# foldl/chatllm.cpp

Measured on AMD Instinct MI355X. Metric: decode tokens/s, higher is better.
Workload: dtype int8xint4 dot / f32 accumulate (Q8_K x Q4_K); 1 GPU; llama3-8b shapes, Q4_K weights, single-token decode, batch 1, 16-token prompt, F16 KV cache; parallelism=single GPU, n_ctx_end=1630

## Files before the change

chatllm.cpp_amd/csrc/common.h:

```cpp
#pragma once

#include <hip/hip_runtime.h>
#include <stdint.h>
#include <stddef.h>

#include "../../include/chatllm_hip.h"
#include "glibc_math.h"
#include "options.h"

#define CLLM_WAVE 64

void cllm_set_error(const char * fmt, ...);
int  cllm_hip_check(hipError_t e, const char * what, const char * file, int line);
#define HIP_TRY(expr) do { int _rc = cllm_hip_check((expr), #expr, __FILE__, __LINE__); if (_rc) return _rc; } while (0)
#define LAUNCH_CHECK() HIP_TRY(hipGetLastError())
#define FAIL(code, ...) do { cllm_set_error(__VA_ARGS__); return (code); } while (0)

#define QK    32
#define QK_K  256
struct __attribute__((packed)) block_q4_0 { uint16_t d; uint8_t qs[16]; };
struct __attribute__((packed)) block_q8_0 { uint16_t d; int8_t  qs[32]; };
struct __attribute__((packed)) block_q4_1 { uint16_t d, m; uint8_t qs[16]; };
struct __attribute__((packed)) block_q8_1 { uint16_t d, s; int8_t  qs[32]; };
struct __attribute__((packed)) block_q4_K { uint16_t d, dmin; uint8_t scales[12]; uint8_t qs[128]; };
// ... 178 lines not shown
__device__ __forceinline__ int   group8_sum_i(int v) { v += dpp_i<DPP_QUAD_XOR1>(v); v += dpp_i<DPP_QUAD_XOR2>(v); return v + dpp_i<DPP_HALF_MIRROR>(v); }
__device__ __forceinline__ int dot4(uint32_t a, uint32_t b, int c) { return __builtin_amdgcn_sdot4((int) a, (int) b, c, false); }
__device__ __forceinline__ void dot4z_x8(const uint32_t (&a)[8], const uint32_t (&b)[8], int (&r)[8]) {
    asm("v_dot4_i32_i8 %0, %8, %16, 0\n\tv_dot4_i32_i8 %1, %9, %17, 0\n\tv_dot4_i32_i8 %2, %10, %18, 0\n\tv_dot4_i32_i8 %3, %11, %19, 0\n\t"
        "v_dot4_i32_i8 %4, %12, %20, 0\n\tv_dot4_i32_i8 %5, %13, %21, 0\n\tv_dot4_i32_i8 %6, %14, %22, 0\n\tv_dot4_i32_i8 %7, %15, %23, 0\n\ts_nop 2"
        : "=&v"(r[0]), "=&v"(r[1]), "=&v"(r[2]), "=&v"(r[3]), "=&v"(r[4]), "=&v"(r[5]), "=&v"(r[6]), "=&v"(r[7])
        : "v"(a[0]), "v"(a[1]), "v"(a[2]), "v"(a[3]), "v"(a[4]), "v"(a[5]), "v"(a[6]), "v"(a[7]),
          "v"(b[0]), "v"(b[1]), "v"(b[2]), "v"(b[3]), "v"(b[4]), "v"(b[5]), "v"(b[6]), "v"(b[7]));
}

static __device__ __noinline__ float libm_expf(float x) { return gm_expf(x); }
static __device__ __noinline__ void rope_cos_sin(float theta, float * c, float * s) {
    *c = gm_cosf(theta);
    *s = gm_sinf(theta);
}

__device__ __forceinline__ float rope_rot_a(float x0, float x1, float c, float s) { return __builtin_fmaf(x0, c, -(x1 * s)); }
__device__ __forceinline__ float rope_rot_b(float x0, float x1, float c, float s) { return __builtin_fmaf(x0, s, x1 * c); }

__device__ __forceinline__ float ggml_expf_poly(float x) {
    const float r = 0x1.8p23f;
    const float z = __builtin_fmaf(x, 0x1.715476p+0f, r);
    const float n = z - r;
    const float b = __builtin_fmaf(-n, 0x1.7f7d1cp-20f, __builtin_fmaf(-n, 0x1.62e4p-1f, x));
    const uint32_t e = __float_as_uint(z) << 23;
    const float k = __uint_as_float(e + 0x3f800000u);
    const bool  c = fabsf(n) > 126.0f;
    const float u = b * b;
    const float j = __builtin_fmaf(__builtin_fmaf(__builtin_fmaf(0x1.0e4020p-7f, b, 0x1.573e2ep-5f), u,
                                                  __builtin_fmaf(0x1.555e66p-3f, b, 0x1.fffdb6p-2f)),
// ... 156 lines not shown
int launch_gemv_decode_tp_gather(hipStream_t st, int wtype, const void * W, int64_t K, int64_t nrows, const float * px, const float * pw, float eps, int epi, float * dst,
                                 const float * bias, const void * ctx_dev, int site, float * xout);
int launch_gemv_rows32(hipStream_t st, int wtype, const void * W, int64_t K, int64_t nrows, int pro, const float * px, const float * pw, float eps, int epi, float * dst, const float * bias, const float * resid);
int gemv_team32_check();
int launch_gemv_team32(hipStream_t st, int wtype, const void * W, int64_t K, int64_t nrows, int pro, const float * px, const float * pw, float eps, int epi, float * dst, const float * bias, const float * resid);
int launch_mmvq_fused(hipStream_t st, int wtype, const void * W, int64_t K, int64_t nrows, int pro, const float * px, const float * pw, float eps, int epi, float * dst, const float * bias, const float * resid);
int launch_attn_decode(hipStream_t st, const float * qkv, const int32_t * pos_dev, int nh, int nkv, int hd, const uint16_t * k_cache, const uint16_t * v_cache, int64_t ML, float * att);
int launch_rope_table(hipStream_t st, const int32_t * pos_dev, int hd, float freq_base, float * cs);
int launch_attn_dec_table(hipStream_t st, const float * qkv, const int32_t * pos_dev, const float * rope_cs, int nh, int nkv, int hd, int mode, uint16_t * k_cache, uint16_t * v_cache, int64_t ML, float * att);
int launch_attn_long(hipStream_t st, const float * qkv, const int32_t * pos_dev, const float * rope_cs, int nh, int nkv, int hd, int mode, uint16_t * k_cache, uint16_t * v_cache, int64_t ML, float * S, float * att);
int launch_gemv_decode_id(hipStream_t st, int wtype, const void * W, size_t w_expert_bytes, int64_t K, int64_t nrows, const float * px, int64_t px_slot_stride,
                          const int32_t * ids, int n_slots, float * dst, int64_t dst_slot_stride, int epi = 0);
int attn_long_threshold();
int launch_rope_kv_attn_decode(hipStream_t st, const float * qkv, const int32_t * pos_dev, int nh, int nkv, int hd, int mode, float freq_base, uint16_t * k_cache, uint16_t * v_cache, int64_t ML, float * att);
int launch_argmax_partial(hipStream_t st, const float * logits, int n, float * part_v, int * part_i);
int launch_argmax_final_next(hipStream_t st, const float * part_v, const int * part_i, int np, int32_t * tok_dev, int32_t * pos_dev, int32_t * out_ring, int32_t * counter,
                             int etype, const void * emb, size_t emb_nb1, int H, float * x_next, int hd, float freq_base, float * cs);
int launch_gemv_rows_argmax(hipStream_t st, const void * W, int64_t K, int64_t nrows, const float * px, const float * pw, float eps, float * dst, float * part_v, int * part_i, int * np);
int launch_argmax_advance(hipStream_t st, const float * logits, int n, int32_t * tok_dev, int32_t * pos_dev, int32_t * out_ring, int32_t * counter, float * part_v, int * part_i);
```

chatllm.cpp_amd/csrc/decode_fused.hip:

```cpp
#include "common.h"
#include "quant_dev.h"
#include "q4k.h"
#include "dequant.h"

#include <math.h>

__device__ __forceinline__ float lane_xor4_ff(float v) { return __int_as_float(lane_xor4_i(__float_as_int(v))); }
__device__ __forceinline__ float vd32_reduce(float a0, float a1) {
    a0 = a0 + dpp_f<DPP_ROW_ROR8>(a0); a1 = a1 + dpp_f<DPP_ROW_ROR8>(a1);
    a0 = a0 + lane_xor4_ff(a0);        a1 = a1 + lane_xor4_ff(a1);
    a0 = a0 + dpp_f<DPP_QUAD_XOR2>(a0); a1 = a1 + dpp_f<DPP_QUAD_XOR2>(a1);
    const float u = a0 + a1;
    return u + dpp_f<DPP_QUAD_XOR1>(u);
}

static float * g_attn_dbg = nullptr;
static unsigned long long * g_attn_ts = nullptr;
extern "C" __attribute__((visibility("default"))) void cllm_debug_set_attn_ts(unsigned long long * dev_buf) { g_attn_ts = dev_buf; }
extern "C" __attribute__((visibility("default"))) void cllm_debug_set_attn_probs(float * dev_buf) { g_attn_dbg = dev_buf; }

template <bool ROPE>
__global__ void __launch_bounds__(1024) k_attn_decode(const float * __restrict__ qkv, const int32_t * __restrict__ pos_dev, int nh, int nkv, int hd,
                                                      float scale, uint16_t * __restrict__ k_cache, uint16_t * __restrict__ v_cache,
                                                      int64_t ML, float * __restrict__ att, float * __restrict__ dbg, int mode, float theta_scale) {
// ... 128 lines not shown
        for (int t = 0; t < 2; t++) {
            const int e = np + 2 * c16 + t;
            if (e < n_kv) tailp[2 * c16 + t] = ((ROPE && e == pos) ? vfresh : h2f(vr[e])) * sc[e];
        }
        wave_lds_fence();
        if (c16 == 0) {
            double s = (double) res;
            for (int t = 0; t < ntail; t++) s += (double) tailp[t];
            att[h * hd + d0] = (float) s;
        }
        wave_lds_fence();
    }
}

__global__ void __launch_bounds__(64) k_rope_table(const int32_t * __restrict__ pos_dev, int half, float theta_scale, float * __restrict__ cs) {
    for (int i = threadIdx.x; i < half; i += 64) {
        float theta = (float) pos_dev[0];
        for (int k = 0; k < i; k++) theta *= theta_scale;
        float c, s_;
        rope_cos_sin(theta, &c, &s_);
        cs[2*i] = c * 1.0f; cs[2*i + 1] = s_ * 1.0f;
    }
}
int launch_rope_table(hipStream_t st, const int32_t * pos_dev, int hd, float freq_base, float * cs) {
    hipLaunchKernelGGL(k_rope_table, dim3(1), dim3(64), 0, st, pos_dev, hd / 2, powf(freq_base, -2.0f / hd), cs);
    LAUNCH_CHECK();
    return CLLM_OK;
}

__device__ __forceinline__ int uniform_load_i32(const int32_t * p) {
    int v;
    asm volatile("s_load_dword %0, %1, 0x0\n\ts_waitcnt lgkmcnt(0)" : "=s"(v) : "s"(p) : "memory");
    return v;
}

template <int HD, int MODE, int PARTS>
__global__ void __launch_bounds__(1024) k_attn_dec(const float * __restrict__ qkv, const int32_t * __restrict__ pos_dev, const float * __restrict__ rope_cs,
// ... 10 lines not shown
    float * qs = sm; float * knew = sm + HD; float * vnew = sm + 2 * HD; float * sc = sm + 3 * HD;

    float px0 = 0.0f, px1 = 0.0f, pc = 0.0f, ps = 0.0f;
    const bool is_pair = tid < 2 * half, is_v = !is_pair && tid < 2 * half + HD;
    const int which = tid >= half ? 1 : 0, pi = tid - which * half, ic = MODE == 0 ? 2 * pi : pi;
    if (is_pair) {
        const float * x = which == 0 ? qkv + h * HD : qkv + QD + g * HD;
        px0 = x[ic]; px1 = x[ic + off];
        pc = rope_cs[2 * pi]; ps = rope_cs[2 * pi + 1];
    } else if (is_v) px0 = qkv[QD + KD + g * HD + (tid - 2 * half)];
    const int pos = uniform_load_i32(pos_dev);
    const int n_kv = pos + 1;
    uint64_t et = 0;
    if (tid >= 992) et = gm_exp2f_T_dev[tid - 992];

    constexpr int NCH = HD / 32, VU = HD / 64 / PARTS, VPF = 8;
    const int vrow0 = PARTS > 1 ? (int) blockIdx.z * VU * 64 : 0;
    const int c16 = lane & 15, sub = lane >> 4;
    const int ib0 = wave * 4 + sub;
    uint32_t kr0[U][NCH];
#pragma unroll
    for (int u = 0; u < U; u++) {
        const int i0 = ib0 + u * 64;
#pragma unroll
        for (int i = 0; i < NCH; i++)
            kr0[u][i] = *(const uint32_t *)(k_cache + (int64_t)(i0 < pos ? i0 : 0) * KD + g * HD + 32 * i + 2 * c16);
    }
    const int np = n_kv & ~31, nch = np >> 5;
    uint32_t vc0[VU][VPF];
#pragma unroll
    for (int u = 0; u < VU; u++) {
        const uint16_t * vr = v_cache + ((int64_t) g * HD + vrow0 + ib0 + u * 64) * ML;
#pragma unroll
        for (int i = 0; i < VPF; i++) vc0[u][i] = *(const uint32_t *)(vr + 32 * (i < nch ? i : 0) + 2 * c16);
    }

    TS(0);
    if (is_pair) {
        const float y0 = rope_rot_a(px0, px1, pc, ps), y1 = rope_rot_b(px0, px1, pc, ps);
        float * o = which == 0 ? qs : knew;
        o[ic] = h2f(f2h(y0)); o[ic + off] = h2f(f2h(y1));
    } else if (is_v) vnew[tid - 2 * half] = h2f(f2h(px0));
    if (tid >= 992) etab_s[tid - 992] = et;
    lds_barrier();
    if (blockIdx.x == 0 && (PARTS == 1 || blockIdx.z == 0) && tid < HD) {
        k_cache[(int64_t) pos * KD + g * HD + tid] = f2h(knew[tid]);
        v_cache[((int64_t) g * HD + tid) * ML + pos] = f2h(vnew[tid]);
    }

// ... 23 lines not shown
                if (c16 == 0 && i0 < pos) sc[i0] = v * scale;
            }
            if (ib + U * 64 < pos) {
#pragma unroll
                for (int u = 0; u < U; u++) {
                    const int i0 = ib + (U + u) * 64;
#pragma unroll
                    for (int i = 0; i < NCH; i++) kr0[u][i] = *(const uint32_t *)(k_cache + (int64_t)(i0 < pos ? i0 : 0) * KD + g * HD + 32 * i + 2 * c16);
                }
            }
        }
    }
    lds_barrier();
    TS(2);

    uint32_t vc1[VU][VPF]; uint16_t vtl[VU][2];
#pragma unroll
    for (int u = 0; u < VU; u++) {
        const uint16_t * vr = v_cache + ((int64_t) g * HD + vrow0 + ib0 + u * 64) * ML;
#pragma unroll
        for (int i = 0; i < VPF; i++) vc1[u][i] = *(const uint32_t *)(vr + 32 * (VPF + i < nch ? VPF + i : 0) + 2 * c16);
#pragma unroll
        for (int t = 0; t < 2; t++) { const int e = np + 2 * c16 + t; vtl[u][t] = vr[e < n_kv ? e : 0]; }
    }
    float mx = -INFINITY;
    for (int i = tid; i < n_kv; i += 1024) mx = fmaxf(mx, sc[i]);
    mx = wave_max(mx);
    if (lane == 0) red_f[wave] = mx;
    lds_barrier();
    mx = red_f[0];
#pragma unroll
    for (int w = 1; w < 16; w++) mx = fmaxf(mx, red_f[w]);
    const int nv = n_kv & ~7;
    for (int i = tid; i < n_kv; i += 1024) {
        const float xv = sc[i] - mx;
        float ev;
        if (i < nv) ev = ggml_expf_poly(xv);
        else { const uint64_t ki = gm_expf_ki(xv); ev = gm_expf_fin(xv, ki, etab_s[ki & 31]); }
// ... 9 lines not shown
        }
        if (lane == 0) for (int i = nv; i < n_kv; i++) sum += (double) sc[i];
        sum = wave_sum_d(sum);
        double rinv = 1.0 / sum;
        if (__builtin_expect(!soft_total_order_safe(rinv, n_kv >> 3), 0)) rinv = 1.0 / soft_sum_serial(sc, nv, n_kv);
        if (lane == 0) red_f[0] = (float) rinv;
    }
    lds_barrier();
    const float inv = red_f[0];
    for (int i = tid; i < n_kv; i += 1024) sc[i] = h2f(f2h(sc[i] * inv));
    lds_barrier();
    TS(3);

    float * tailp = sc + ML + (wave * 4 + sub) * 32;
    const int ntail = n_kv - np;
#pragma unroll
    for (int u = 0; u < VU; u++) {
        const int d0 = vrow0 + ib0 + u * 64;
        const uint16_t * vr = v_cache + ((int64_t) g * HD + d0) * ML;
        const float vfresh = vnew[d0];
        float a0 = 0.0f, a1 = 0.0f;
        auto chunk = [&](uint32_t w, int ci) {
            const int e = 32 * ci + 2 * c16;
            typedef float f32x2_t __attribute__((ext_vector_type(2)));
            const f32x2_t pr = *(const f32x2_t *)(sc + e);
            const float v0 = e == pos ? vfresh : h2f((uint16_t)(w & 0xffff)), v1 = e + 1 == pos ? vfresh : h2f((uint16_t)(w >> 16));
            a0 = __builtin_fmaf(v0, pr.x, a0); a1 = __builtin_fmaf(v1, pr.y, a1);
        };
#pragma unroll
        for (int i = 0; i < VPF; i++) if (i < nch) chunk(vc0[u][i], i);
        if (nch > VPF) {
#pragma unroll
            for (int i = 0; i < VPF; i++) if (VPF + i < nch) chunk(vc1[u][i], VPF + i);
#pragma clang loop unroll(disable)
            for (int c8 = 2 * VPF; c8 < nch; c8 += VPF) {
                uint32_t w[VPF];
#pragma unroll
                for (int i = 0; i < VPF; i++) w[i] = *(const uint32_t *)(vr + 32 * (c8 + i < nch ? c8 + i : 0) + 2 * c16);
#pragma unroll
                for (int i = 0; i < VPF; i++) if (c8 + i < nch) chunk(w[i], c8 + i);
            }
        }
        const float res = vd32_reduce(a0, a1);
#pragma unroll
        for (int t = 0; t < 2; t++) {
            const int e = np + 2 * c16 + t;
            if (e < n_kv) tailp[2 * c16 + t] = (e == pos ? vfresh : h2f(vtl[u][t])) * sc[e];
        }
        wave_lds_fence();
        if (c16 == 0) {
            double s = (double) res;
            for (int t = 0; t < ntail; t++) s += (double) tailp[t];
            att[h * HD + d0] = (float) s;
        }
        wave_lds_fence();
    }
    TS(4);
#undef TS
}

int launch_attn_dec_table(hipStream_t st, const float * qkv, const int32_t * pos_dev, const float * rope_cs, int nh, int nkv, int hd, int mode,
                          uint16_t * k_cache, uint16_t * v_cache, int64_t ML, float * att) {
    if ((hd != 64 && hd != 128) || nh % nkv || ML % 8 || ML > (1 << 30) || g_attn_dbg) return CLLM_E_UNSUPPORTED;
    const size_t lds = (size_t)(3 * hd + ML) * 4 + 64 * 32 * 4;
    if (lds > 150 * 1024) return CLLM_E_UNSUPPORTED;
    const float scale = 1.0f / sqrtf((float) hd);
    const dim3 grid(nh / nkv, nkv, hd == 128 ? 2 : 1);
#define GO(HD_, MODE_) do { \
        static uint64_t attr = 0; \
        if (lds > 48 * 1024 && dev_flag_unset(attr)) { HIP_TRY(hipFuncSetAttribute((const void *) k_attn_dec<HD_, MODE_, (HD_ == 128 ? 2 : 1)>, hipFuncAttributeMaxDynamicSharedMemorySize, 150 * 1024)); dev_flag_set(attr); } \
        hipLaunchKernelGGL((k_attn_dec<HD_, MODE_, (HD_ == 128 ? 2 : 1)>), grid, dim3(1024), lds, st, qkv, pos_dev, rope_cs, nh, nkv, scale, k_cache, v_cache, (int) ML, att, g_attn_ts); } while (0)
    if (hd == 128) { if (mode == 0) GO(128, 0); else GO(128, 2); }
    else           { if (mode == 0) GO(64, 0);  else GO(64, 2); }
#undef GO
    LAUNCH_CHECK();
    return CLLM_OK;
}

static int attn_launch(hipStream_t st, bool rope, const float * qkv, const int32_t * pos_dev, int nh, int nkv, int hd, uint16_t * k_cache, uint16_t * v_cache,
                       int64_t ML, float * att, int mode, float freq_base) {
    if (hd % 8 || (ML % 8) || nh % nkv) FAIL(CLLM_E_UNSUPPORTED, "attn_decode: head_dim and max_len must be multiples of 8");
    const size_t lds = (size_t)(3 * hd + (ML > hd ? ML : hd)) * 4 + 64 * 32 * 4;
    if (lds > 150 * 1024) FAIL(CLLM_E_UNSUPPORTED, "attn_decode: max_len %lld does not fit LDS", (long long) ML);
    static uint64_t attr0 = 0, attr1 = 0;
    if (lds > 48 * 1024) {
        if (!rope && dev_flag_unset(attr0)) { HIP_TRY(hipFuncSetAttribute((const void *) k_attn_decode<false>, hipFuncAttributeMaxDynamicSharedMemorySize, 150 * 1024)); dev_flag_set(attr0); }
// ... 75 lines not shown
    float best = -INFINITY; int idx = 0x7fffffff;
    for (int i = threadIdx.x; i < np; i += 256) argmax_combine(best, idx, pv[i], pi[i]);
#pragma unroll
    for (int o = 32; o > 0; o >>= 1) argmax_combine(best, idx, __shfl_xor(best, o, 64), __shfl_xor(idx, o, 64));
    if ((threadIdx.x & 63) == 0) { bv[threadIdx.x >> 6] = best; bi[threadIdx.x >> 6] = idx; }
    __syncthreads();
    if (threadIdx.x == 0) {
        for (int w = 1; w < 4; w++) argmax_combine(best, idx, bv[w], bi[w]);
        if (idx == 0x7fffffff) idx = 0;
        tok_dev[0] = idx;
        pos_dev[0] = pos_dev[0] + 1;
        out_ring[counter[0]] = idx;
        counter[0] = counter[0] + 1;
    }
}
__global__ void __launch_bounds__(1024) k_argmax_final_next(const float * __restrict__ pv, const int * __restrict__ pi, int np, int32_t * __restrict__ tok_dev,
                                                            int32_t * __restrict__ pos_dev, int32_t * __restrict__ out_ring, int32_t * __restrict__ counter,
                                                            int etype, const char * __restrict__ emb, size_t emb_nb1, int H, float * __restrict__ x_next,
                                                            int half, float theta_scale, float * __restrict__ cs) {
    __shared__ float bv[16]; __shared__ int bi[16]; __shared__ int tok_s;
    const int tid = threadIdx.x;
    const int pos_next = pos_dev[0] + 1;
    float best = -INFINITY; int idx = 0x7fffffff;
    for (int i = tid; i < np; i += 1024) argmax_combine(best, idx, pv[i], pi[i]);
#pragma unroll
    for (int o = 32; o > 0; o >>= 1) argmax_combine(best, idx, __shfl_xor(best, o, 64), __shfl_xor(idx, o, 64));
    if ((tid & 63) == 0) { bv[tid >> 6] = best; bi[tid >> 6] = idx; }
    __syncthreads();
    if (tid == 0) {
        for (int w = 1; w < 16; w++) argmax_combine(best, idx, bv[w], bi[w]);
        if (idx == 0x7fffffff) idx = 0;
        tok_s = idx;
        tok_dev[0] = idx;
        pos_dev[0] = pos_next;
        out_ring[counter[0]] = idx;
        counter[0] = counter[0] + 1;
    }
    if (cs && tid >= 960)
        for (int i = tid - 960; i < half; i += 64) {
            float theta = (float) pos_next;
            for (int k = 0; k < i; k++) theta *= theta_scale;
            float c, s_;
            rope_cos_sin(theta, &c, &s_);
            cs[2*i] = c * 1.0f; cs[2*i + 1] = s_ * 1.0f;
        }
    __syncthreads();
    const char * row = emb + (size_t) tok_s * emb_nb1;
    for (int c = tid; c < H; c += 1024) x_next[c] = dequant_elem(etype, row, c);
}
int launch_argmax_partial(hipStream_t st, const float * logits, int n, float * part_v, int * part_i) {
    hipLaunchKernelGGL(k_argmax_partial, dim3(256), dim3(256), 0, st, logits, n, part_v, part_i);
    LAUNCH_CHECK();
    return CLLM_OK;
}
int launch_argmax_final_next(hipStream_t st, const float * part_v, const int * part_i, int np, int32_t * tok_dev, int32_t * pos_dev, int32_t * out_ring, int32_t * counter,
                             int etype, const void * emb, size_t emb_nb1, int H, float * x_next, int hd, float freq_base, float * cs) {
    hipLaunchKernelGGL(k_argmax_final_next, dim3(1), dim3(1024), 0, st, part_v, part_i, np, tok_dev, pos_dev, out_ring, counter, etype, (const char *) emb, emb_nb1, H, x_next,
                       hd / 2, hd ? powf(freq_base, -2.0f / hd) : 0.0f, hd ? cs : (float *) nullptr);
    LAUNCH_CHECK();
    return CLLM_OK;
}
__global__ void __launch_bounds__(256) k_argmax_publish(const float * __restrict__ pv, const int * __restrict__ pi, int np, int32_t * __restrict__ tok_dev,
                                                        int32_t * __restrict__ tok_host, int32_t * const * __restrict__ inc, int n_inc) {
    __shared__ float bv[4]; __shared__ int bi[4];
    float best = -INFINITY; int idx = 0x7fffffff;
    for (int i = threadIdx.x; i < np; i += 256) argmax_combine(best, idx, pv[i], pi[i]);
#pragma unroll
    for (int o = 32; o > 0; o >>= 1) argmax_combine(best, idx, __shfl_xor(best, o, 64), __shfl_xor(idx, o, 64));
    if ((threadIdx.x & 63) == 0) { bv[threadIdx.x >> 6] = best; bi[threadIdx.x >> 6] = idx; }
    __syncthreads();
    if (threadIdx.x == 0) {
        for (int w = 1; w < 4; w++) argmax_combine(best, idx, bv[w], bi[w]);
        if (idx == 0x7fffffff) idx = 0;
// ... 108 lines not shown
```

chatllm.cpp_amd/csrc/decoder.hip:

```cpp
#include "common.h"

#include <string>
#include <vector>
#include <map>
#include <math.h>
#include <string.h>
#include <stdio.h>

struct dweight { int type = -1; void * data = nullptr; size_t bytes = 0; bool owned = false; };

struct llama_layer {
    dweight attn_norm, ffn_norm, wq, wk, wv, wo, wgate, wup, wdown, bq, bk, bv;
    dweight wqkv, wgu;
    dweight bqkv;
    uint16_t * k_cache = nullptr, * v_cache = nullptr;
};

struct cllm_llama {
    cllm_llama_config cfg;
    hipStream_t st = nullptr;
    int nh = 0, nkv = 0, F = 0;
    dweight tok_embd, lm_head, out_norm;
    std::vector<llama_layer> layers;
    bool finalized = false;
// ... 510 lines not shown
        TRY(norm_gemv(L.wgu, 2*F, (const float *) L.ffn_norm.data, silu_epi ? 1 : 0, silu_epi ? m->g : m->gu, nullptr));
        if (!tp) TRY(launch_mmvq_fused(st, L.wdown.type, L.wdown.data, F, H, dpro, dsrc, nullptr, 0.0f, 0, xc, nullptr, xc));
        else if (fused_ar) {
            const int rc = launch_gemv_decode_tp_scatter(st, L.wdown.type, L.wdown.data, F, H, dpro, dsrc, fctx, 2 * il + 1);
            if (rc == CLLM_E_UNSUPPORTED) FAIL(CLLM_E_UNSUPPORTED, "decode: the fused all-reduce cannot take down_proj (type %d, K %lld); unbind it (cllm_llama_set_tp_fused(m, NULL))", L.wdown.type, (long long) F);
            if (rc) return rc;
            pend_site = 2 * il + 1;
        } else {
            TRY(launch_mmvq_fused(st, L.wdown.type, L.wdown.data, F, H, dpro, dsrc, nullptr, 0.0f, 0, m->o, nullptr, nullptr));
            TRY(tp_allreduce(m, st, m->o, H));
            pend = m->o;
        }
    }
    float * part_v = (float *)(m->counter_dev + 16); int * part_i = (int *)(m->counter_dev + 16 + 256);
    if (sample && !head) {
        int np = 256, rc = CLLM_E_UNSUPPORTED;
        if (pend_site < 0 && !pend && m->lm_head.type == CLLM_TYPE_Q4_K)
            rc = launch_gemv_rows_argmax(st, m->lm_head.data, H, V, xc, (const float *) m->out_norm.data, c.rms_eps, m->logits, part_v, part_i, &np);
        if (rc == CLLM_E_UNSUPPORTED) {
            TRY(norm_gemv(m->lm_head, V, (const float *) m->out_norm.data, 0, m->logits, nullptr));
            TRY(launch_argmax_partial(st, m->logits, (int) V, part_v, part_i));
            np = 256;
        } else if (rc) return rc;
        TRY(launch_argmax_final_next(st, part_v, part_i, np, m->tokens_dev, m->pos_dev, m->out_ring, m->counter_dev, m->tok_embd.type, m->tok_embd.data,
                                     cllm_row_size(m->tok_embd.type, H), (int) H, m->x, cs_table ? (int) hd : 0, c.rope_theta, rope_cs));
        return CLLM_OK;
    }
    TRY(norm_gemv(m->lm_head, V, (const float *) m->out_norm.data, 0, m->logits, nullptr));
    if (sample) TRY(launch_argmax_advance(st, m->logits, (int) V, m->tokens_dev, m->pos_dev, m->out_ring, m->counter_dev, part_v, part_i));
    return CLLM_OK;
}

static int kernel_wait_check(cllm_llama * m) {
    TRY(gemv_team32_check());
    if (m->tp_oneshot && cllm_tp_oneshot_error(m->tp_oneshot)) FAIL(CLLM_E_HIP, "decode: a flag wait of the one-shot all-reduce timed out (a peer rank is late, dead or out of step): the step's logits are void");
    if (m->tp_fused && cllm_tp_fused_error(m->tp_fused)) FAIL(CLLM_E_HIP, "decode: a granule wait of the fused all-reduce timed out (a peer rank is late, dead or out of step): the step's logits are void");
    return CLLM_OK;
}

static int ensure_decode_graph(cllm_llama * m, bool long_ctx) {
// ... 92 lines not shown
    if (!m->fused_ok) FAIL(CLLM_E_UNSUPPORTED, "decode_fused_logits: this model/config cannot take the fused path");
    const int32_t init[2] = { token, n_past };
    HIP_TRY(hipMemcpyAsync(m->tokens_dev, &init[0], 4, hipMemcpyHostToDevice, m->st));
    HIP_TRY(hipMemcpyAsync(m->pos_dev, &init[1], 4, hipMemcpyHostToDevice, m->st));
    HIP_TRY(hipStreamSynchronize(m->st));
    TRY(ensure_scores(m, (size_t) m->nh * m->cfg.max_len * 3 / 2 + 64));
    TRY(decode_step_fused(m, false, n_past + 1 > attn_long_threshold()));
    HIP_TRY(hipMemcpyAsync(logits_host, m->logits, (size_t) m->cfg.vocab * 4, hipMemcpyDeviceToHost, m->st));
    HIP_TRY(hipStreamSynchronize(m->st));
    return kernel_wait_check(m);
}

extern "C" int cllm_llama_debug_read(cllm_llama * m, const char * what, float * host, int64_t n) {
    if (!m || !what || !host || n <= 0) FAIL(CLLM_E_INVALID, "debug_read: arguments");
    const std::string w(what);
    const float * src = w == "x" ? m->x : w == "qkv" ? m->qkv : w == "att" ? m->att : w == "gu" ? m->gu : w == "logits" ? m->logits : nullptr;
    if (!src) FAIL(CLLM_E_INVALID, "debug_read: unknown buffer '%s'", what);
    HIP_TRY(hipMemcpyAsync(host, src, (size_t) n * 4, hipMemcpyDeviceToHost, m->st));
    HIP_TRY(hipStreamSynchronize(m->st));
    return CLLM_OK;
}
```

chatllm.cpp_amd/csrc/gemv_rows.hip:

```cpp
#include "common.h"
#include "quant_dev.h"
#include "q4k.h"

#define ROWS_SLOT_BYTES 2304
#ifndef ROWS_NS
#define ROWS_NS 3
#endif

__device__ __forceinline__ float silu_poly_r(float x) { return x / (1.0f + ggml_expf_poly(0.0f - x)); }
__device__ __forceinline__ float silu_any_r(float x, bool body) { return body ? silu_poly_r(x) : x / (1.0f + libm_expf(-x)); }

__device__ __forceinline__ void dma16(const char * base , unsigned voff, unsigned lds_dst ) {
    unsigned keep;
#ifdef ROWS_NT
    asm volatile("s_mov_b32 %0, m0\n\ts_mov_b32 m0, %3\n\ts_nop 0\n\tglobal_load_lds_dwordx4 %1, %2 nt\n\ts_mov_b32 m0, %0" : "=&s"(keep) : "v"(voff), "s"(base), "s"(lds_dst) : "memory");
#else
    asm volatile("s_mov_b32 %0, m0\n\ts_mov_b32 m0, %3\n\ts_nop 0\n\tglobal_load_lds_dwordx4 %1, %2\n\ts_mov_b32 m0, %0" : "=&s"(keep) : "v"(voff), "s"(base), "s"(lds_dst) : "memory");
#endif
}
template <int N> __device__ __forceinline__ void wait_vm() { asm volatile("s_waitcnt vmcnt(%0)" :: "n"(N) : "memory"); }

template <int PRO, int EPI, int NPRE, int RPW>
__global__ void __launch_bounds__(1024) k_gemv_rows(const float * __restrict__ px, const float * __restrict__ pw, const char * __restrict__ W, int nblk, int nunits, float eps,
                                                    float * __restrict__ dst, const float * __restrict__ bias, const float * resid) {
    extern __shared__ __attribute__((aligned(16))) char lds[];
    constexpr int GPR = 8 / RPW;
    constexpr int CPR = ROWS_SLOT_BYTES / RPW / 16;
    constexpr int BPS = 2 * GPR;
    constexpr int NS = ROWS_NS;
    const int tid = threadIdx.x, lane = tid & 63;
    const int K = nblk * 256;
    const unsigned nb01 = (unsigned) nblk * 144u;

    const float * gp = (PRO == 1 || PRO == 4) ? pw : PRO == 3 ? px + 4 : px;
    constexpr int vmul = PRO == 3 ? 2 : 1;
    const int e0 = tid * 4;
    f32x4 vv[NPRE], gg[NPRE];
#pragma unroll
    for (int u = 0; u < NPRE; u++) {
// ... 46 lines not shown
            if (PRO == 3) {
                const f32x4 p0 = vv[u], p1 = gg[u];
                v.x = silu_any_r(p0.x, e + 0 < nv) * p0.y; v.y = silu_any_r(p0.z, e + 1 < nv) * p0.w;
                v.z = silu_any_r(p1.x, e + 2 < nv) * p1.y; v.w = silu_any_r(p1.z, e + 3 < nv) * p1.w;
            }
            if (PRO == 4) {
                const f32x4 g = gg[u];
                v.x = silu_any_r(v.x, e + 0 < nv) * g.x; v.y = silu_any_r(v.y, e + 1 < nv) * g.y; v.z = silu_any_r(v.z, e + 2 < nv) * g.z; v.w = silu_any_r(v.w, e + 3 < nv) * g.w;
            }
            if (PRO == 1) { const f32x4 g = gg[u]; v.x = (v.x * scale) * g.x; v.y = (v.y * scale) * g.y; v.z = (v.z * scale) * g.z; v.w = (v.w * scale) * g.w; }
            quant4_store<256, false>(lds, K, e, lane, v);
        }
    }
    __syncthreads();
    if (EPI != 2 && nmine == 0) return;

    const int j = lane & 7;
    const int A = 4 * (j & 1) + (j & 2) + (j >> 2);
    const int kk = ((j & 1) << 1) | ((j >> 1) & 1);
    const int rowg = RPW == 8 ? lane >> 3 : lane >> 4;
    const int gg2 = RPW == 8 ? 0 : (lane >> 3) & 1;
    const bool hi = gg2 != 0;
    const unsigned lrow = ring + (unsigned) rowg * (CPR * 16u) + (unsigned) gg2 * 144u + 16u + 4u * A;
    const unsigned lhdr = ring + (unsigned) rowg * (CPR * 16u) + (unsigned) gg2 * 144u;
    const char * act = lds;
    const float * actd = (const float *)(lds + act_off_d(K));
    const int * acts = (const int *)(lds + act_off_s(K, 256));
    typedef __attribute__((address_space(3))) const uint32_t * lptr;
    typedef __attribute__((address_space(3))) const u32x4 * lptr4;

// ... 79 lines not shown
            const float ov = __shfl_xor(bestv, o, 64); const int oi = __shfl_xor(besti, o, 64);
            if (ov > bestv || (ov == bestv && oi < besti)) { bestv = ov; besti = oi; }
        }
        __syncthreads();
        float * lv = (float *) lds; int * li = (int *)(lds + 64);
        if (lane == 0) { lv[wave] = bestv; li[wave] = besti; }
        __syncthreads();
        if (tid == 0) {
            for (int w = 1; w < 16; w++) { const float ov = lv[w]; const int oi = li[w]; if (ov > bestv || (ov == bestv && oi < besti)) { bestv = ov; besti = oi; } }
            ((float *) bias)[blockIdx.x] = bestv; ((int *) resid)[blockIdx.x] = besti;
        }
    }
}

static int gemv_rows_go(hipStream_t st, const void * W, int64_t K, int64_t nrows, int pro, const float * px, const float * pw, float eps, int epi, float * dst,
                        const float * bias, const float * resid, int * grid_out) {
    static const int mode = opt_int(OPT_CLLM_GEMV_ROWS);
    if (!mode || K % 256 || pro < 1 || pro > 4 || nrows <= 0 || (uint64_t) nrows * (uint64_t)(K / 256 * 144) >= (1ull << 32)) return CLLM_E_UNSUPPORTED;
    if (K > ((pro == 2 || pro == 4) ? 32768 : 16384)) return CLLM_E_UNSUPPORTED;
    if (epi == 1 && (pro != 1 || bias || resid)) return CLLM_E_UNSUPPORTED;
    if (epi == 2 && (pro != 1 || !bias || !resid)) return CLLM_E_UNSUPPORTED;
    const int nblk = (int)(K / 256), cus = device_cu_count();
    if (mode == 1 && nrows / 8 < 32 * (int64_t) cus) return CLLM_E_UNSUPPORTED;
    int rpw = mode == 8 || mode == 4 ? mode : (nrows / 8 >= 8 * (int64_t) cus ? 8 : 4);
    if (rpw == 8 && (nblk % 2 || nrows % 8)) rpw = 4;
    if (rpw == 4 && (nblk % 4 || nrows % 4)) { if (nblk % 2 == 0 && nrows % 8 == 0) rpw = 8; else return CLLM_E_UNSUPPORTED; }
    if (epi == 1 && nrows % (2 * rpw)) return CLLM_E_UNSUPPORTED;
    const int nunits = (int)(nrows / rpw);
    int grid = nunits < cus ? nunits : cus;
    if (epi == 2 && grid > 256) return CLLM_E_UNSUPPORTED;
    const size_t lds = act_row_bytes(K, 256) + 16 * (size_t) ROWS_NS * ROWS_SLOT_BYTES;
    if (lds > 159 * 1024) return CLLM_E_UNSUPPORTED;
    const int npre = K <= 4096 ? 1 : K <= 16384 ? 4 : 8;
#define GOR(PRO_, EPI_, NPRE_, RPW_) do { \
        static uint64_t attr = 0; \
        if (dev_flag_unset(attr)) { HIP_TRY(hipFuncSetAttribute((const void *) k_gemv_rows<PRO_, EPI_, NPRE_, RPW_>, hipFuncAttributeMaxDynamicSharedMemorySize, 159 * 1024)); dev_flag_set(attr); } \
        hipLaunchKernelGGL((k_gemv_rows<PRO_, EPI_, NPRE_, RPW_>), dim3((unsigned) grid), dim3(1024), lds, st, px, pw, (const char *) W, nblk, nunits, eps, dst, bias, resid); } while (0)
#define GOP(RPW_) do { \
        if (pro == 1 && epi == 1) { if (npre == 1) GOR(1, 1, 1, RPW_); else GOR(1, 1, 4, RPW_); } \
        else if (pro == 1 && epi == 2) { if (npre == 1) GOR(1, 2, 1, RPW_); else GOR(1, 2, 4, RPW_); } \
        else if (pro == 1)        { if (npre == 1) GOR(1, 0, 1, RPW_); else GOR(1, 0, 4, RPW_); } \
        else if (pro == 2)        { if (npre == 1) GOR(2, 0, 1, RPW_); else if (npre == 4) GOR(2, 0, 4, RPW_); else GOR(2, 0, 8, RPW_); } \
        else if (pro == 4)        { if (npre == 1) GOR(4, 0, 1, RPW_); else if (npre == 4) GOR(4, 0, 4, RPW_); else GOR(4, 0, 8, RPW_); } \
        else                      { if (npre == 1) GOR(3, 0, 1, RPW_); else GOR(3, 0, 4, RPW_); } } while (0)
    if (rpw == 8) GOP(8); else GOP(4);
#undef GOP
#undef GOR
    LAUNCH_CHECK();
    if (grid_out) *grid_out = grid;
    return CLLM_OK;
}
int launch_gemv_rows(hipStream_t st, const void * W, int64_t K, int64_t nrows, int pro, const float * px, const float * pw, float eps, int epi, float * dst,
                     const float * bias, const float * resid) {
    if (epi != 0 && epi != 1) return CLLM_E_UNSUPPORTED;
    return gemv_rows_go(st, W, K, nrows, pro, px, pw, eps, epi, dst, bias, resid, nullptr);
}
int launch_gemv_rows_argmax(hipStream_t st, const void * W, int64_t K, int64_t nrows, const float * px, const float * pw, float eps, float * dst, float * part_v, int * part_i, int * np) {
    if (!part_v || !part_i || !np || nrows > INT32_MAX) return CLLM_E_UNSUPPORTED;
    return gemv_rows_go(st, W, K, nrows, 1, px, pw, eps, 2, dst, (const float *) part_v, (const float *) part_i, np);
}
```

Before: 669.2 tokens/s.

## Move next-token rope table into lm_head kernel and split attention into more parts

Builds the next position's rope cos/sin table inside the lm_head gemv-argmax kernel (in the last block's spare wave) or in an extra block of the argmax-partial kernel. This takes it off the serial single-block argmax_final kernel. That kernel is also slimmed: it drops its LDS reduction and barriers, loads partials directly per lane, and specialises on Q4_K embedding dequant. Separately, attention decode for hd=128 splits V rows across 8 parts instead of 2 to spread work over more blocks. The catch is that some waves now sit idle and K/score work is recomputed per part.

```diff
diff --git a/chatllm.cpp_amd/csrc/common.h b/chatllm.cpp_amd/csrc/common.h
--- a/chatllm.cpp_amd/csrc/common.h
+++ b/chatllm.cpp_amd/csrc/common.h
@@ -216,6 +216,16 @@
     *c = gm_cosf(theta);
     *s = gm_sinf(theta);
 }
+__device__ __forceinline__ void rope_table_wave(int pos, int half, float theta_scale, float * __restrict__ cs, int lane) {
+    for (int i = lane; i < half; i += 64) {
+        float theta = (float) pos;
+        for (int k = 0; k < i; k++) theta *= theta_scale;
+        float c, s_;
+        rope_cos_sin(theta, &c, &s_);
+        cs[2*i] = c * 1.0f; cs[2*i + 1] = s_ * 1.0f;
+    }
+}
+struct rope_next { const int32_t * pos_dev; float * cs; int half; float theta_scale; };
 
 __device__ __forceinline__ float rope_rot_a(float x0, float x1, float c, float s) { return __builtin_fmaf(x0, c, -(x1 * s)); }
 __device__ __forceinline__ float rope_rot_b(float x0, float x1, float c, float s) { return __builtin_fmaf(x0, s, x1 * c); }
@@ -402,7 +412,10 @@
 int attn_long_threshold();
 int launch_rope_kv_attn_decode(hipStream_t st, const float * qkv, const int32_t * pos_dev, int nh, int nkv, int hd, int mode, float freq_base, uint16_t * k_cache, uint16_t * v_cache, int64_t ML, float * att);
 int launch_argmax_partial(hipStream_t st, const float * logits, int n, float * part_v, int * part_i);
+rope_next rope_next_args(const int32_t * pos_dev, int hd, float freq_base, float * cs);
+int launch_argmax_partial_next(hipStream_t st, const float * logits, int n, float * part_v, int * part_i, rope_next nx);
 int launch_argmax_final_next(hipStream_t st, const float * part_v, const int * part_i, int np, int32_t * tok_dev, int32_t * pos_dev, int32_t * out_ring, int32_t * counter,
-                             int etype, const void * emb, size_t emb_nb1, int H, float * x_next, int hd, float freq_base, float * cs);
-int launch_gemv_rows_argmax(hipStream_t st, const void * W, int64_t K, int64_t nrows, const float * px, const float * pw, float eps, float * dst, float * part_v, int * part_i, int * np);
+                             int etype, const void * emb, size_t emb_nb1, int H, float * x_next);
+int launch_gemv_rows_argmax(hipStream_t st, const void * W, int64_t K, int64_t nrows, const float * px, const float * pw, float eps, float * dst, float * part_v, int * part_i, int * np,
+                            rope_next nx);
 int launch_argmax_advance(hipStream_t st, const float * logits, int n, int32_t * tok_dev, int32_t * pos_dev, int32_t * out_ring, int32_t * counter, float * part_v, int * part_i);
diff --git a/chatllm.cpp_amd/csrc/decode_fused.hip b/chatllm.cpp_amd/csrc/decode_fused.hip
--- a/chatllm.cpp_amd/csrc/decode_fused.hip
+++ b/chatllm.cpp_amd/csrc/decode_fused.hip
@@ -166,13 +166,7 @@
 }
 
 __global__ void __launch_bounds__(64) k_rope_table(const int32_t * __restrict__ pos_dev, int half, float theta_scale, float * __restrict__ cs) {
-    for (int i = threadIdx.x; i < half; i += 64) {
-        float theta = (float) pos_dev[0];
-        for (int k = 0; k < i; k++) theta *= theta_scale;
-        float c, s_;
-        rope_cos_sin(theta, &c, &s_);
-        cs[2*i] = c * 1.0f; cs[2*i + 1] = s_ * 1.0f;
-    }
+    rope_table_wave(pos_dev[0], half, theta_scale, cs, threadIdx.x);
 }
 int launch_rope_table(hipStream_t st, const int32_t * pos_dev, int hd, float freq_base, float * cs) {
     hipLaunchKernelGGL(k_rope_table, dim3(1), dim3(64), 0, st, pos_dev, hd / 2, powf(freq_base, -2.0f / hd), cs);
@@ -213,8 +207,10 @@
     uint64_t et = 0;
     if (tid >= 992) et = gm_exp2f_T_dev[tid - 992];
 
-    constexpr int NCH = HD / 32, VU = HD / 64 / PARTS, VPF = 8;
-    const int vrow0 = PARTS > 1 ? (int) blockIdx.z * VU * 64 : 0;
+    constexpr int NCH = HD / 32, RP = HD / PARTS, VU = RP >= 64 ? RP / 64 : 1, VPF = RP >= 64 ? 8 : 16;
+    static_assert(RP % 4 == 0 && RP * PARTS == HD && (RP >= 64 ? RP % 64 == 0 : true), "rows per part: whole waves of four lane groups");
+    const int vrow0 = PARTS > 1 ? (int) blockIdx.z * RP : 0;
+    const bool vrow = RP >= 64 || __builtin_amdgcn_readfirstlane(wave) < RP / 4;
     const int c16 = lane & 15, sub = lane >> 4;
     const int ib0 = wave * 4 + sub;
     uint32_t kr0[U][NCH];
@@ -227,11 +223,13 @@
     }
     const int np = n_kv & ~31, nch = np >> 5;
     uint32_t vc0[VU][VPF];
-#pragma unroll
-    for (int u = 0; u < VU; u++) {
-        const uint16_t * vr = v_cache + ((int64_t) g * HD + vrow0 + ib0 + u * 64) * ML;
-#pragma unroll
-        for (int i = 0; i < VPF; i++) vc0[u][i] = *(const uint32_t *)(vr + 32 * (i < nch ? i : 0) + 2 * c16);
+    if (vrow) {
+#pragma unroll
+        for (int u = 0; u < VU; u++) {
+            const uint16_t * vr = v_cache + ((int64_t) g * HD + vrow0 + ib0 + u * 64) * ML;
+#pragma unroll
+            for (int i = 0; i < VPF; i++) vc0[u][i] = *(const uint32_t *)(vr + 32 * (i < nch ? i : 0) + 2 * c16);
+        }
     }
 
     TS(0);
@@ -285,14 +283,19 @@
     lds_barrier();
     TS(2);
 
-    uint32_t vc1[VU][VPF]; uint16_t vtl[VU][2];
-#pragma unroll
-    for (int u = 0; u < VU; u++) {
-        const uint16_t * vr = v_cache + ((int64_t) g * HD + vrow0 + ib0 + u * 64) * ML;
-#pragma unroll
-        for (int i = 0; i < VPF; i++) vc1[u][i] = *(const uint32_t *)(vr + 32 * (VPF + i < nch ? VPF + i : 0) + 2 * c16);
-#pragma unroll
-        for (int t = 0; t < 2; t++) { const int e = np + 2 * c16 + t; vtl[u][t] = vr[e < n_kv ? e : 0]; }
+    constexpr int VPF1 = VPF < 16 ? VPF : 1;
+    uint32_t vc1[VU][VPF1]; uint16_t vtl[VU][2];
+    if (vrow) {
+#pragma unroll
+        for (int u = 0; u < VU; u++) {
+            const uint16_t * vr = v_cache + ((int64_t) g * HD + vrow0 + ib0 + u * 64) * ML;
+            if constexpr (VPF < 16) {
+#pragma unroll
+                for (int i = 0; i < VPF; i++) vc1[u][i] = *(const uint32_t *)(vr + 32 * (VPF + i < nch ? VPF + i : 0) + 2 * c16);
+            }
+#pragma unroll
+            for (int t = 0; t < 2; t++) { const int e = np + 2 * c16 + t; vtl[u][t] = vr[e < n_kv ? e : 0]; }
+        }
     }
     float mx = -INFINITY;
     for (int i = tid; i < n_kv; i += 1024) mx = fmaxf(mx, sc[i]);
@@ -332,6 +335,7 @@
 
     float * tailp = sc + ML + (wave * 4 + sub) * 32;
     const int ntail = n_kv - np;
+    if (vrow) {
 #pragma unroll
     for (int u = 0; u < VU; u++) {
         const int d0 = vrow0 + ib0 + u * 64;
@@ -348,15 +352,17 @@
 #pragma unroll
         for (int i = 0; i < VPF; i++) if (i < nch) chunk(vc0[u][i], i);
         if (nch > VPF) {
-#pragma unroll
-            for (int i = 0; i < VPF; i++) if (VPF + i < nch) chunk(vc1[u][i], VPF + i);
+            if constexpr (VPF < 16) {
+#pragma unroll
+                for (int i = 0; i < VPF; i++) if (VPF + i < nch) chunk(vc1[u][i], VPF + i);
+            }
 #pragma clang loop unroll(disable)
-            for (int c8 = 2 * VPF; c8 < nch; c8 += VPF) {
-                uint32_t w[VPF];
-#pragma unroll
-                for (int i = 0; i < VPF; i++) w[i] = *(const uint32_t *)(vr + 32 * (c8 + i < nch ? c8 + i : 0) + 2 * c16);
-#pragma unroll
-                for (int i = 0; i < VPF; i++) if (c8 + i < nch) chunk(w[i], c8 + i);
+            for (int c8 = 16; c8 < nch; c8 += 8) {
+                uint32_t w[8];
+#pragma unroll
+                for (int i = 0; i < 8; i++) w[i] = *(const uint32_t *)(vr + 32 * (c8 + i < nch ? c8 + i : 0) + 2 * c16);
+#pragma unroll
+                for (int i = 0; i < 8; i++) if (c8 + i < nch) chunk(w[i], c8 + i);
             }
         }
         const float res = vd32_reduce(a0, a1);
@@ -373,21 +379,25 @@
         }
         wave_lds_fence();
     }
+    }
     TS(4);
 #undef TS
 }
 
+#ifndef ATTN_PARTS_128
+#define ATTN_PARTS_128 8
+#endif
 int launch_attn_dec_table(hipStream_t st, const float * qkv, const int32_t * pos_dev, const float * rope_cs, int nh, int nkv, int hd, int mode,
                           uint16_t * k_cache, uint16_t * v_cache, int64_t ML, float * att) {
     if ((hd != 64 && hd != 128) || nh % nkv || ML % 8 || ML > (1 << 30) || g_attn_dbg) return CLLM_E_UNSUPPORTED;
     const size_t lds = (size_t)(3 * hd + ML) * 4 + 64 * 32 * 4;
     if (lds > 150 * 1024) return CLLM_E_UNSUPPORTED;
     const float scale = 1.0f / sqrtf((float) hd);
-    const dim3 grid(nh / nkv, nkv, hd == 128 ? 2 : 1);
+    const dim3 grid(nh / nkv, nkv, hd == 128 ? ATTN_PARTS_128 : 1);
 #define GO(HD_, MODE_) do { \
         static uint64_t attr = 0; \
-        if (lds > 48 * 1024 && dev_flag_unset(attr)) { HIP_TRY(hipFuncSetAttribute((const void *) k_attn_dec<HD_, MODE_, (HD_ == 128 ? 2 : 1)>, hipFuncAttributeMaxDynamicSharedMemorySize, 150 * 1024)); dev_flag_set(attr); } \
-        hipLaunchKernelGGL((k_attn_dec<HD_, MODE_, (HD_ == 128 ? 2 : 1)>), grid, dim3(1024), lds, st, qkv, pos_dev, rope_cs, nh, nkv, scale, k_cache, v_cache, (int) ML, att, g_attn_ts); } while (0)
+        if (lds > 48 * 1024 && dev_flag_unset(attr)) { HIP_TRY(hipFuncSetAttribute((const void *) k_attn_dec<HD_, MODE_, (HD_ == 128 ? ATTN_PARTS_128 : 1)>, hipFuncAttributeMaxDynamicSharedMemorySize, 150 * 1024)); dev_flag_set(attr); } \
+        hipLaunchKernelGGL((k_attn_dec<HD_, MODE_, (HD_ == 128 ? ATTN_PARTS_128 : 1)>), grid, dim3(1024), lds, st, qkv, pos_dev, rope_cs, nh, nkv, scale, k_cache, v_cache, (int) ML, att, g_attn_ts); } while (0)
     if (hd == 128) { if (mode == 0) GO(128, 0); else GO(128, 2); }
     else           { if (mode == 0) GO(64, 0);  else GO(64, 2); }
 #undef GO
@@ -493,39 +503,63 @@
         counter[0] = counter[0] + 1;
     }
 }
+__global__ void __launch_bounds__(256) k_argmax_partial_next(const float * __restrict__ x, int n, float * __restrict__ pv, int * __restrict__ pi, rope_next nx) {
+    __shared__ float bv[4]; __shared__ int bi[4];
+    const int nb = gridDim.x - 1;
+    if ((int) blockIdx.x == nb) {
+        if (threadIdx.x < 64) rope_table_wave(nx.pos_dev[0] + 1, nx.half, nx.theta_scale, nx.cs, threadIdx.x);
+        return;
+    }
+    const int per = (n + nb - 1) / nb;
+    const int lo = blockIdx.x * per, hi = min(n, lo + per);
+    float best = -INFINITY; int idx = 0x7fffffff;
+    for (int i = lo + threadIdx.x; i < hi; i += 256) { const float v = x[i]; if (v > best) { best = v; idx = i; } }
+#pragma unroll
+    for (int o = 32; o > 0; o >>= 1) argmax_combine(best, idx, __shfl_xor(best, o, 64), __shfl_xor(idx, o, 64));
+    if ((threadIdx.x & 63) == 0) { bv[threadIdx.x >> 6] = best; bi[threadIdx.x >> 6] = idx; }
+    __syncthreads();
+    if (threadIdx.x == 0) {
+        for (int w = 1; w < 4; w++) argmax_combine(best, idx, bv[w], bi[w]);
+        pv[blockIdx.x] = best; pi[blockIdx.x] = idx;
+    }
+}
+rope_next rope_next_args(const int32_t * pos_dev, int hd, float freq_base, float * cs) {
+    rope_next nx;
+    nx.pos_dev = pos_dev; nx.cs = hd ? cs : (float *) nullptr; nx.half = hd / 2; nx.theta_scale = hd ? powf(freq_base, -2.0f / hd) : 0.0f;
+    return nx;
+}
+int launch_argmax_partial_next(hipStream_t st, const float * logits, int n, float * part_v, int * part_i, rope_next nx) {
+    if (!nx.cs) return launch_argmax_partial(st, logits, n, part_v, part_i);
+    hipLaunchKernelGGL(k_argmax_partial_next, dim3(257), dim3(256), 0, st, logits, n, part_v, part_i, nx);
+    LAUNCH_CHECK();
+    return CLLM_OK;
+}
+template <int ETYPE>
 __global__ void __launch_bounds__(1024) k_argmax_final_next(const float * __restrict__ pv, const int * __restrict__ pi, int np, int32_t * __restrict__ tok_dev,
                                                             int32_t * __restrict__ pos_dev, int32_t * __restrict__ out_ring, int32_t * __restrict__ counter,
-                                                            int etype, const char * __restrict__ emb, size_t emb_nb1, int H, float * __restrict__ x_next,
-                                                            int half, float theta_scale, float * __restrict__ cs) {
-    __shared__ float bv[16]; __shared__ int bi[16]; __shared__ int tok_s;
-    const int tid = threadIdx.x;
-    const int pos_next = pos_dev[0] + 1;
+                                                            int etype, const char * __restrict__ emb, size_t emb_nb1, int H, float * __restrict__ x_next) {
+    const int tid = threadIdx.x, lane = tid & 63;
+    int pos = 0, cnt = 0;
+    if (tid == 0) { pos = pos_dev[0]; cnt = counter[0]; }
+    float pvv[4]; int pii[4];
+#pragma unroll
+    for (int k = 0; k < 4; k++) { const int i = lane + 64 * k, ic = i < np ? i : 0; pvv[k] = pv[ic]; pii[k] = pi[ic]; }
     float best = -INFINITY; int idx = 0x7fffffff;
-    for (int i = tid; i < np; i += 1024) argmax_combine(best, idx, pv[i], pi[i]);
-#pragma unroll
-    for (int o = 32; o > 0; o >>= 1) argmax_combine(best, idx, __shfl_xor(best, o, 64), __shfl_xor(idx, o, 64));
-    if ((tid & 63) == 0) { bv[tid >> 6] = best; bi[tid >> 6] = idx; }
-    __syncthreads();
+#pragma unroll
+    for (int k = 0; k < 4; k++) if (lane + 64 * k < np) argmax_combine(best, idx, pvv[k], pii[k]);
+#pragma unroll
+    for (int o = 32; o > 0; o >>= 1) argmax_combine(best, idx, __shfl_xor(best, o, 64), __shfl_xor(idx, o, 64));
+    if (idx == 0x7fffffff) idx = 0;
+    idx = __builtin_amdgcn_readfirstlane(idx);
+    const char * row = emb + (size_t) idx * emb_nb1;
+    const int ty = ETYPE >= 0 ? ETYPE : etype;
+    for (int c = tid; c < H; c += 1024) x_next[c] = dequant_elem(ty, row, c);
     if (tid == 0) {
-        for (int w = 1; w < 16; w++) argmax_combine(best, idx, bv[w], bi[w]);
-        if (idx == 0x7fffffff) idx = 0;
-        tok_s = idx;
         tok_dev[0] = idx;
-        pos_dev[0] = pos_next;
-        out_ring[counter[0]] = idx;
-        counter[0] = counter[0] + 1;
-    }
-    if (cs && tid >= 960)
-        for (int i = tid - 960; i < half; i += 64) {
-            float theta = (float) pos_next;
-            for (int k = 0; k < i; k++) theta *= theta_scale;
-            float c, s_;
-            rope_cos_sin(theta, &c, &s_);
-            cs[2*i] = c * 1.0f; cs[2*i + 1] = s_ * 1.0f;
-        }
-    __syncthreads();
-    const char * row = emb + (size_t) tok_s * emb_nb1;
-    for (int c = tid; c < H; c += 1024) x_next[c] = dequant_elem(etype, row, c);
+        pos_dev[0] = pos + 1;
+        out_ring[cnt] = idx;
+        counter[0] = cnt + 1;
+    }
 }
 int launch_argmax_partial(hipStream_t st, const float * logits, int n, float * part_v, int * part_i) {
     hipLaunchKernelGGL(k_argmax_partial, dim3(256), dim3(256), 0, st, logits, n, part_v, part_i);
@@ -533,9 +567,12 @@
     return CLLM_OK;
 }
 int launch_argmax_final_next(hipStream_t st, const float * part_v, const int * part_i, int np, int32_t * tok_dev, int32_t * pos_dev, int32_t * out_ring, int32_t * counter,
-                             int etype, const void * emb, size_t emb_nb1, int H, float * x_next, int hd, float freq_base, float * cs) {
-    hipLaunchKernelGGL(k_argmax_final_next, dim3(1), dim3(1024), 0, st, part_v, part_i, np, tok_dev, pos_dev, out_ring, counter, etype, (const char *) emb, emb_nb1, H, x_next,
-                       hd / 2, hd ? powf(freq_base, -2.0f / hd) : 0.0f, hd ? cs : (float *) nullptr);
+                             int etype, const void * emb, size_t emb_nb1, int H, float * x_next) {
+    if (np < 1 || np > 256) FAIL(CLLM_E_INVALID, "argmax_final_next: %d partials (1..256)", np);
+    if (etype == CLLM_TYPE_Q4_K)
+        hipLaunchKernelGGL(k_argmax_final_next<CLLM_TYPE_Q4_K>, dim3(1), dim3(1024), 0, st, part_v, part_i, np, tok_dev, pos_dev, out_ring, counter, etype, (const char *) emb, emb_nb1, H, x_next);
+    else
+        hipLaunchKernelGGL(k_argmax_final_next<-1>, dim3(1), dim3(1024), 0, st, part_v, part_i, np, tok_dev, pos_dev, out_ring, counter, etype, (const char *) emb, emb_nb1, H, x_next);
     LAUNCH_CHECK();
     return CLLM_OK;
 }
diff --git a/chatllm.cpp_amd/csrc/decoder.hip b/chatllm.cpp_amd/csrc/decoder.hip
--- a/chatllm.cpp_amd/csrc/decoder.hip
+++ b/chatllm.cpp_amd/csrc/decoder.hip
@@ -548,16 +548,17 @@
     }
     float * part_v = (float *)(m->counter_dev + 16); int * part_i = (int *)(m->counter_dev + 16 + 256);
     if (sample && !head) {
+        const rope_next nx = rope_next_args(m->pos_dev, cs_table ? (int) hd : 0, c.rope_theta, rope_cs);
         int np = 256, rc = CLLM_E_UNSUPPORTED;
         if (pend_site < 0 && !pend && m->lm_head.type == CLLM_TYPE_Q4_K)
-            rc = launch_gemv_rows_argmax(st, m->lm_head.data, H, V, xc, (const float *) m->out_norm.data, c.rms_eps, m->logits, part_v, part_i, &np);
+            rc = launch_gemv_rows_argmax(st, m->lm_head.data, H, V, xc, (const float *) m->out_norm.data, c.rms_eps, m->logits, part_v, part_i, &np, nx);
         if (rc == CLLM_E_UNSUPPORTED) {
             TRY(norm_gemv(m->lm_head, V, (const float *) m->out_norm.data, 0, m->logits, nullptr));
-            TRY(launch_argmax_partial(st, m->logits, (int) V, part_v, part_i));
+            TRY(launch_argmax_partial_next(st, m->logits, (int) V, part_v, part_i, nx));
             np = 256;
         } else if (rc) return rc;
         TRY(launch_argmax_final_next(st, part_v, part_i, np, m->tokens_dev, m->pos_dev, m->out_ring, m->counter_dev, m->tok_embd.type, m->tok_embd.data,
-                                     cllm_row_size(m->tok_embd.type, H), (int) H, m->x, cs_table ? (int) hd : 0, c.rope_theta, rope_cs));
+                                     cllm_row_size(m->tok_embd.type, H), (int) H, m->x));
         return CLLM_OK;
     }
     TRY(norm_gemv(m->lm_head, V, (const float *) m->out_norm.data, 0, m->logits, nullptr));
@@ -680,8 +681,10 @@
 extern "C" int cllm_llama_debug_read(cllm_llama * m, const char * what, float * host, int64_t n) {
     if (!m || !what || !host || n <= 0) FAIL(CLLM_E_INVALID, "debug_read: arguments");
     const std::string w(what);
-    const float * src = w == "x" ? m->x : w == "qkv" ? m->qkv : w == "att" ? m->att : w == "gu" ? m->gu : w == "logits" ? m->logits : nullptr;
+    const float * src = w == "x" ? m->x : w == "qkv" ? m->qkv : w == "att" ? m->att : w == "gu" ? m->gu : w == "logits" ? m->logits :
+                        w == "rope_cs" ? (const float *)(m->counter_dev + 16 + 512) : nullptr;
     if (!src) FAIL(CLLM_E_INVALID, "debug_read: unknown buffer '%s'", what);
+    if (w == "rope_cs" && n > 512) FAIL(CLLM_E_INVALID, "debug_read: the cos / sin table holds at most 512 values");
     HIP_TRY(hipMemcpyAsync(host, src, (size_t) n * 4, hipMemcpyDeviceToHost, m->st));
     HIP_TRY(hipStreamSynchronize(m->st));
     return CLLM_OK;
diff --git a/chatllm.cpp_amd/csrc/gemv_rows.hip b/chatllm.cpp_amd/csrc/gemv_rows.hip
--- a/chatllm.cpp_amd/csrc/gemv_rows.hip
+++ b/chatllm.cpp_amd/csrc/gemv_rows.hip
@@ -22,7 +22,7 @@
 
 template <int PRO, int EPI, int NPRE, int RPW>
 __global__ void __launch_bounds__(1024) k_gemv_rows(const float * __restrict__ px, const float * __restrict__ pw, const char * __restrict__ W, int nblk, int nunits, float eps,
-                                                    float * __restrict__ dst, const float * __restrict__ bias, const float * resid) {
+                                                    float * __restrict__ dst, const float * __restrict__ bias, const float * resid, rope_next nx) {
     extern __shared__ __attribute__((aligned(16))) char lds[];
     constexpr int GPR = 8 / RPW;
     constexpr int CPR = ROWS_SLOT_BYTES / RPW / 16;
@@ -99,6 +99,7 @@
     }
     __syncthreads();
     if (EPI != 2 && nmine == 0) return;
+    if (EPI == 2 && nx.cs && blockIdx.x == gridDim.x - 1 && wave == 15) rope_table_wave(nx.pos_dev[0] + 1, nx.half, nx.theta_scale, nx.cs, lane);
 
     const int j = lane & 7;
     const int A = 4 * (j & 1) + (j & 2) + (j >> 2);
@@ -208,7 +209,7 @@
 }
 
 static int gemv_rows_go(hipStream_t st, const void * W, int64_t K, int64_t nrows, int pro, const float * px, const float * pw, float eps, int epi, float * dst,
-                        const float * bias, const float * resid, int * grid_out) {
+                        const float * bias, const float * resid, int * grid_out, rope_next nx = rope_next{nullptr, nullptr, 0, 0.0f}) {
     static const int mode = opt_int(OPT_CLLM_GEMV_ROWS);
     if (!mode || K % 256 || pro < 1 || pro > 4 || nrows <= 0 || (uint64_t) nrows * (uint64_t)(K / 256 * 144) >= (1ull << 32)) return CLLM_E_UNSUPPORTED;
     if (K > ((pro == 2 || pro == 4) ? 32768 : 16384)) return CLLM_E_UNSUPPORTED;
@@ -229,7 +230,7 @@
 #define GOR(PRO_, EPI_, NPRE_, RPW_) do { \
         static uint64_t attr = 0; \
         if (dev_flag_unset(attr)) { HIP_TRY(hipFuncSetAttribute((const void *) k_gemv_rows<PRO_, EPI_, NPRE_, RPW_>, hipFuncAttributeMaxDynamicSharedMemorySize, 159 * 1024)); dev_flag_set(attr); } \
-        hipLaunchKernelGGL((k_gemv_rows<PRO_, EPI_, NPRE_, RPW_>), dim3((unsigned) grid), dim3(1024), lds, st, px, pw, (const char *) W, nblk, nunits, eps, dst, bias, resid); } while (0)
+        hipLaunchKernelGGL((k_gemv_rows<PRO_, EPI_, NPRE_, RPW_>), dim3((unsigned) grid), dim3(1024), lds, st, px, pw, (const char *) W, nblk, nunits, eps, dst, bias, resid, nx); } while (0)
 #define GOP(RPW_) do { \
         if (pro == 1 && epi == 1) { if (npre == 1) GOR(1, 1, 1, RPW_); else GOR(1, 1, 4, RPW_); } \
         else if (pro == 1 && epi == 2) { if (npre == 1) GOR(1, 2, 1, RPW_); else GOR(1, 2, 4, RPW_); } \
@@ -249,7 +250,8 @@
     if (epi != 0 && epi != 1) return CLLM_E_UNSUPPORTED;
     return gemv_rows_go(st, W, K, nrows, pro, px, pw, eps, epi, dst, bias, resid, nullptr);
 }
-int launch_gemv_rows_argmax(hipStream_t st, const void * W, int64_t K, int64_t nrows, const float * px, const float * pw, float eps, float * dst, float * part_v, int * part_i, int * np) {
+int launch_gemv_rows_argmax(hipStream_t st, const void * W, int64_t K, int64_t nrows, const float * px, const float * pw, float eps, float * dst, float * part_v, int * part_i, int * np,
+                            rope_next nx) {
     if (!part_v || !part_i || !np || nrows > INT32_MAX) return CLLM_E_UNSUPPORTED;
-    return gemv_rows_go(st, W, K, nrows, 1, px, pw, eps, 2, dst, (const float *) part_v, (const float *) part_i, np);
-}
+    return gemv_rows_go(st, W, K, nrows, 1, px, pw, eps, 2, dst, (const float *) part_v, (const float *) part_i, np, nx);
+}
```

Measured after the change: 674.1 tokens/s (median of 6 runs). Within noise of the previous version (+0.7%).
